# tensorchord/VectorChord-bm25

Hardware: AMD Instinct MI355X
Metric: queries/sec top-10 BM25, 10M synthetic docs; achieved HBM GB/s vs peak (higher is better)
Workload: dtype f64

## Files before the change

vectorchord-bm25_amd/api.py:

```python
import ctypes as C

import numpy as np

from ._lib import IndexDesc, SynthParams, Vbm25Error, check, lib

HIT_DTYPE = np.dtype({"names": ["score", "doc_id", "payload"],
                      "formats": ["<f8", "<u4", ("<u2", (3,))],
                      "offsets": [0, 8, 12], "itemsize": 24})

WIDTH = 16

_DESC_ARRAYS = [
    ("term_key", np.uint8), ("term_df", np.uint32), ("term_wand_fn", np.uint8),
    ("term_wand_tf", np.uint32), ("term_first_block", np.uint32), ("blk_min_doc", np.uint32),
    ("blk_max_doc", np.uint32), ("blk_n", np.uint8), ("blk_wand_fn", np.uint8),
    ("blk_wand_tf", np.uint32), ("blk_meta_doc", np.uint8), ("blk_meta_tf", np.uint8),
    ("blk_off8", np.uint32), ("blob", np.uint8), ("doc_fieldnorm", np.uint8),
    ("doc_payload", np.uint16),
]


def _p(a):
    return a.ctypes.data_as(C.c_void_p) if a is not None and a.size else None

# ... 333 lines not shown
            check(lib().vbm25_batch_set_filter(self.h, None, None))
            self.doc_filter = None
            return
        sel = np.full(self.max_queries, NO_FILTER, dtype=np.uint32)
        if q_filter is not None:
            q_filter = np.asarray(q_filter, dtype=np.uint32).reshape(-1)
            if len(q_filter) > self.max_queries:
                raise ValueError(f"{len(q_filter)} selectors for a batch of {self.max_queries} queries")
            sel[:len(q_filter)] = q_filter
        check(lib().vbm25_batch_set_filter(self.h, doc_filter.h, _p(sel)))
        self.doc_filter = doc_filter

    def set_growing(self, growing):
        check(lib().vbm25_batch_set_growing(self.h, growing.h if growing is not None else None))
        self.growing = growing

    def device_results(self):
        hits, n_hits = C.c_void_p(), C.c_void_p()
        check(lib().vbm25_batch_device_results(self.h, C.byref(hits), C.byref(n_hits)))
        return hits.value, n_hits.value

    def kernel_ms(self):
        ms, n = C.c_double(), C.c_uint32()
        check(lib().vbm25_batch_kernel_ms(self.h, C.byref(ms), C.byref(n)))
        return ms.value, n.value

    def debug_counts(self):
        f = lib().vbm25_batch_debug_counts
        f.restype = C.c_int
        f.argtypes = [C.c_void_p, C.c_void_p, C.c_void_p]
        ni, nf = C.c_uint32(), C.c_uint32()
        check(f(self.h, C.byref(ni), C.byref(nf)))
        return ni.value, nf.value

    def debug_route(self):
        f = lib().vbm25_batch_debug_route
        f.restype = C.c_int
        f.argtypes = [C.c_void_p]
        return int(f(self.h))

    def debug_routes(self):
        f = lib().vbm25_batch_debug_routes
        f.restype = C.c_int
        f.argtypes = [C.c_void_p, C.c_void_p]
        out = (C.c_uint32 * 6)()
        check(f(self.h, out))
        return tuple(int(x) for x in out)

    def debug_win_launches(self):
        f = lib().vbm25_batch_debug_win_launches
        f.restype = C.c_int
        f.argtypes = [C.c_void_p]
        return int(f(self.h))

    def debug_theta(self, nq):
        f = getattr(lib(), "vbm25_batch_debug_theta", None)
        if f is None:
            return None
        f.restype = C.c_int
        f.argtypes = [C.c_void_p, C.c_void_p]
        out = np.zeros(nq, dtype=np.uint64)
        check(f(self.h, out.ctypes.data))
        return out.view(np.float64)

    def debug_check(self):
        f = getattr(lib(), "vbm25_batch_debug_check", None)
        if f is None:
            return None
        f.restype = C.c_int
        f.argtypes = [C.c_void_p, C.c_void_p]
        out = (C.c_uint32 * 16)()
        check(f(self.h, out))
        return tuple(int(x) for x in out)


class Stream:

    def __init__(self, index, depth, max_queries, max_total_terms, k):
        self.index, self.k = index, k
        self.h = C.c_void_p()
        L = lib()
        check(L.vbm25_stream_create(index.h, depth, max_queries, max(1, max_total_terms), k, C.byref(self.h)))
        self._nq = []
        self.growing = None
        self.doc_filter = None
        self._held = []

    def __del__(self):
        try:
            if self.h:
                lib().vbm25_stream_destroy(self.h)
        except Exception:
            pass

    def set_growing(self, growing):
        check(lib().vbm25_stream_set_growing(self.h, growing.h if growing is not None else None))
        self.growing = growing

    def set_filter(self, doc_filter):
        check(lib().vbm25_stream_set_filter(self.h, doc_filter.h if doc_filter is not None else None))
        self.doc_filter = doc_filter

    def submit(self, term_ids, q_off, q_filter=None):
        term_ids = np.ascontiguousarray(term_ids, dtype=np.uint32)
        q_off = np.ascontiguousarray(q_off, dtype=np.uint32)
        nq = len(q_off) - 1
# ... 534 lines not shown
```

vectorchord-bm25_amd/csrc/scan_win.h:

```cpp

#pragma clang diagnostic push
#pragma clang diagnostic ignored "-Winline-asm"
constexpr int WN_T = 8;
#ifndef VBM25_WIN_WAVES_MAX
#define VBM25_WIN_WAVES_MAX 12
#endif
constexpr int wn_wave_lds(int mt) { return 8192 + 512 * mt + 256; }
constexpr int wn_waves(int mt, int rk) {
    const int by_lds = (163840 - 2048) / wn_wave_lds(mt);
    const int by_regs = (rk == 1 && mt <= 5) || (rk == 2 && mt <= 4) ? 16 : 12;
    const int n = by_lds < by_regs ? by_lds : by_regs;
    return n < VBM25_WIN_WAVES_MAX ? n : VBM25_WIN_WAVES_MAX;
}
constexpr int WN_BM_WORDS = 2048;
constexpr int WN_SLOT = 256;
constexpr int WN_LIST = 64;
constexpr uint32_t WN_GRID = 256;

typedef __attribute__((address_space(3))) uint32_t wn_lds_u32;
struct WnBm {
    uint32_t base, mask;
};
__device__ __forceinline__ uint32_t wn_or_rtn(const WnBm bm, const uint32_t x, const uint32_t bit) {
    return __hip_atomic_fetch_or((wn_lds_u32 *)(((x >> 3) & bm.mask) | bm.base), bit, __ATOMIC_RELAXED, __HIP_MEMORY_SCOPE_WORKGROUP);
// ... 171 lines not shown
                nsv += (uint32_t)__popcll(hm);
                continue;
            }
            if (ranked) {
                ranked = false;
                __builtin_amdgcn_wave_barrier();
                const bool hb = lane < nsv;
                rtop.offer(hb, hb ? sv_score[lane] : 0.0, hb ? sv_doc[lane] : 0u, k, lane);
            }
            rtop.offer(has, sc, d, k, lane);
        }
        __builtin_amdgcn_wave_barrier();
    }
    auto emit = [&](uint32_t i, double sc, uint32_t d) {
        const uint16_t *pl = ix.doc_payload + 3ull * d;
        unsigned long long *out = reinterpret_cast<unsigned long long *>(ca->bt.hits + (size_t)q * k + i);
        out[0] = (unsigned long long)__double_as_longlong(sc);
        out[1] = (unsigned long long)d | (unsigned long long)pl[0] << 32 | (unsigned long long)pl[1] << 48;
        out[2] = (unsigned long long)pl[2];
    };
    uint32_t n;
    if (ranked) {
        __builtin_amdgcn_wave_barrier();
        const bool mine = lane < nsv;
        const double sc = mine ? sv_score[lane] : 0.0;
        const uint32_t d = mine ? sv_doc[lane] : 0u;
        uint32_t place = 0;
        for (uint32_t j = 0; j < nsv; ++j) {
            const double sj = readlane_f64(sc, j);
            const uint32_t dj = (uint32_t)__builtin_amdgcn_readlane((int)d, (int)j);
            place += better(sj, dj, sc, d) ? 1u : 0u;
        }
        n = min(nsv, k);
        if (mine && place < k) emit(place, sc, d);
    } else {
        n = rtop.cnt;
#pragma unroll
        for (int r = 0; r < RK; ++r)
            if (r * 64 + lane < n) emit(r * 64 + lane, rtop.score[r], rtop.doc[r]);
    }
    uint32_t nf = 0;
    for (uint32_t i = lane; i < g; i += 64) {
        nf += __hip_atomic_load(&ca->bt.item_failed[L0 + i], __ATOMIC_RELAXED, __HIP_MEMORY_SCOPE_AGENT) != 0u ? 1u : 0u;
        __hip_atomic_store(&ca->bt.item_failed[L0 + i], 0u, __ATOMIC_RELAXED, __HIP_MEMORY_SCOPE_AGENT);
        __hip_atomic_store(&ca->bt.res_cnt[L0 + i], 0u, __ATOMIC_RELAXED, __HIP_MEMORY_SCOPE_AGENT);
    }
#pragma unroll
    for (int o = 32; o > 0; o >>= 1) nf += __shfl_xor(nf, o);
    if (lane == 0) {
        ca->bt.n_hits[q] = nf ? NONE32 : n;
        ca->bt.q_failed[q] = nf;
        ca->bt.theta_last[q] = theta;
        __hip_atomic_store(&ca->bt.theta[q], 0ull, __ATOMIC_RELAXED, __HIP_MEMORY_SCOPE_AGENT);
        __hip_atomic_store(&ca->bt.fused_state[1 + q], 0u, __ATOMIC_RELAXED, __HIP_MEMORY_SCOPE_AGENT);
    }
}

template <int MT, int RK, bool FILT>
__global__ void __launch_bounds__(wn_waves(MT, RK) * 64, (wn_waves(MT, RK) + 3) / 4) scan_win_kernel(DevIndex ix, DevBatch bt) {
    constexpr int WN_WAVES = wn_waves(MT, RK), WN_WG = WN_WAVES * 64;
    static_assert(sizeof(WinWave<MT>) + WN_BM_WORDS * 4 == wn_wave_lds(MT), "wn_waves() knows the size");
    __shared__ alignas(8192) uint32_t BM[WN_WAVES * WN_BM_WORDS];
    __shared__ WinWave<MT> SW[WN_WAVES];
    __shared__ double S1[256];
    const uint32_t lane = threadIdx.x & 63;
    WinWave<MT> &S = SW[uni(threadIdx.x >> 6)];
    uint32_t *const bm = &BM[uni(threadIdx.x >> 6) * WN_BM_WORDS];
    WnBm bmbase;
    bmbase.base = uni((uint32_t)(uintptr_t)(wn_lds_u32 *)bm);
    bmbase.mask = 0x1ffcu;
    asm volatile("" : "+v"(bmbase.mask));
    const uint32_t k = bt.k, g = bt.win_g, n_items = bt.nq * g, NWIN = ix.n_win;
#ifdef VBM25_DEV
    const uint32_t dbg = bt.win_dbg;
#else
    constexpr uint32_t dbg = 0;
#endif
    const uint16_t *ids16 = reinterpret_cast<const uint16_t *>(ix.post_id16);
    for (uint32_t i = threadIdx.x; i < 256u; i += WN_WG) S1[i] = ix.s1[i];
#pragma unroll
    for (int i = 0; i < WN_BM_WORDS / 4 / 64; ++i) reinterpret_cast<uint4 *>(bm)[lane + 64 * i] = make_uint4(0, 0, 0, 0);
    __syncthreads();
#ifdef VBM25_PROFILE
    unsigned long long prof[16] = {0, 0, 0, 0, 0, 0, 0, 0, 0, 0, 0, 0, 0, 0, 0, 0};
    const unsigned long long prof_t0 = __builtin_readcyclecounter();
#endif

    const uint32_t n_waves = gridDim.x * (uint32_t)WN_WAVES;
    uint32_t drawn = blockIdx.x * (uint32_t)WN_WAVES + uni(threadIdx.x >> 6);
    uint32_t merge_q = NONE32;
    if (dbg & 8u) {
        uint32_t d0 = 0;
        if (lane == 0) d0 = atomicAdd(cold_args()->bt.work_ctr, 1u);
        drawn = uni(d0);
    }
    for (;;) {
        uint32_t item = drawn;
        if (item >= n_items) break;
        uint32_t w_lo, w_hi;
        {
            const KernArgsP ca = cold_args();
            const uint32_t oo = ca->bt.order_on;
            if (oo == 1u) item = uni(ca->bt.item_order[item]);
            else if (oo == 2u) {
                const uint32_t full12 = (ca->bt.nq >> 2) * 12u;
                if (item < full12) {
                    const uint32_t wgi = item / 12u, r = item - wgi * 12u;
                    item = (wgi * 4u + (r & 3u)) * 3u + (r >> 2);
                }
            }
        }
        PROF_T(t_item);
        const uint32_t q = item / g, part = item - q * g;
        {
            const KernArgsP ca = cold_args();
            if (g <= 16u && ca->bt.win_cut[g] != 0u) {
                w_lo = ca->bt.win_cut[part];
                w_hi = ca->bt.win_cut[part + 1u];
            } else {
                w_lo = (uint32_t)((unsigned long long)NWIN * part / g);
                w_hi = (uint32_t)((unsigned long long)NWIN * (part + 1u) / g);
            }
        }

        uint32_t m = 0, term = NONE32;
        uint32_t fbi = NONE32;
        {
            const KernArgsP ca = cold_args();
            const uint32_t qs = ca->bt.q_stride;
            const uint32_t qb = qs ? qs * q : uni(ca->bt.q_off[q]), qe = qs ? qs * (q + 1u) : uni(ca->bt.q_off[q + 1]);
            const uint32_t *idfb = ca->bt.id16_fb;
            const uint32_t tt = lane < qe - qb ? ca->bt.term_ids[qb + lane] : NONE32;
            const uint32_t ti = idfb && lane < qe - qb ? idfb[qb + lane] : NONE32;
            const bool ok = tt < ix.n_terms;
            const unsigned long long okm = __ballot(ok);
            if (ok) {
                S.list[wn_mbcnt(okm)] = tt;
                if (wn_mbcnt(okm) < 32u) S.list[32u + wn_mbcnt(okm)] = ti;
            }
            m = (uint32_t)__popcll(okm);
            __builtin_amdgcn_wave_barrier();
            if (lane < min(m, (uint32_t)MT)) {
                term = S.list[lane];
                fbi = S.list[32u + lane];
            }
            __builtin_amdgcn_wave_barrier();
        }
        const bool act = lane < min(m, (uint32_t)MT);
        uint32_t fb = 0, wb = 0;
        double s0 = 0.0, kth = 0.0;
        {
            const KernArgsP ca = cold_args();
            const double *kub = ca->ix.term_kth_ub;
            if constexpr (FILT)
                if (query_filter(q)) kub = nullptr;
            if (act) {
                fb = ca->ix.term_first_block[term];
                if (fbi == NONE32) fbi = fb;
                s0 = ca->ix.term_s0[term];
                wb = ca->ix.term_win[term];
                if (kub) {
// ... 405 lines not shown
                        wn_wait_all(pb.gw);
                        c2(pb);
                    }
                    pb.found = false;
                    c1(pb, epp, nd1, w);
                    pb.valid = true;
                }
            }
#ifdef VBM25_WIN_WIPE_STORES
            if (!(dbg & 64u))
#pragma unroll
                for (int i = 0; i < WN_BM_WORDS / 4 / 64; ++i) reinterpret_cast<uint4 *>(bm)[lane + 64 * i] = make_uint4(0, 0, 0, 0);
#else
            if (!(dbg & 64u)) {
#define WN_WIPE4(o) "ds_write_addtid_b32 %1 offset:" #o "\n\tds_write_addtid_b32 %1 offset:" #o "+256\n\tds_write_addtid_b32 %1 offset:" #o "+512\n\tds_write_addtid_b32 %1 offset:" #o "+768\n\t"
#define WN_WIPE32(o) WN_WIPE4(o) WN_WIPE4(o + 1024) WN_WIPE4(o + 2048) WN_WIPE4(o + 3072) WN_WIPE4(o + 4096) WN_WIPE4(o + 5120) WN_WIPE4(o + 6144) WN_WIPE4(o + 7168)
                asm volatile("s_mov_b32 m0, %0\n\ts_nop 0\n\t" WN_WIPE32(0) : : "s"(bmbase.base), "v"(vzero) : "m0", "memory");
#undef WN_WIPE32
#undef WN_WIPE4
            }
#endif
            PROF_T(t_5);
            PROF_ADD(7, t_w2, t_5);
            {
                wn_wait_theta<MT>(pgv);
                const unsigned long long pg = ((unsigned long long)uni((uint32_t)(pgv >> 32)) << 32) | uni((uint32_t)pgv);
                if (pg > th) th = pg;
            }
            wn_load_theta(pgv, vzero, &bt.theta[q]);
            c1_request(pa);
            c1_request(pb);
            load_runs(cur, w - w_lo + 2u);
            PROF_T(t_6);
            PROF_ADD(11, t_5, t_6);
            if (failed) return false;
            return true;
        };
        PROF_T(t_loop);
        for (uint32_t w = w_lo; w < w_hi; w += 2u) {
            if (!window(bufa, w)) break;
            if (w + 1u < w_hi && !window(bufb, w + 1u)) break;
        }
        PROF_T(t_loop_end);
        double cold_ub[MT];
#pragma unroll
        for (int t = 0; t < MT; ++t) {
            const uint32_t pS = (uint32_t)__builtin_amdgcn_readlane((int)wS, t), pE = (uint32_t)__builtin_amdgcn_readlane((int)wE, t);
            const uint32_t fbt = (uint32_t)__builtin_amdgcn_readlane((int)fb, t);
            const bool in = (uint32_t)t < mm && pE != pS && (pS >> 7) + lane <= ((pE - 1u) >> 7);
            cold_ub[t] = in ? ix.blk_ub[fbt + (pS >> 7) + lane] : 0.0;
        }
        wn_drain<MT>(bufa, bufb, pa.gw, pb.gw, pgv);
        uint32_t next_draw = n_items;
        if (lane == 0 && n_items > n_waves) next_draw = atomicAdd(cold_args()->bt.work_ctr, 1u);
        if (pa.valid && !failed) c2(pa);
        if (pb.valid && !failed) c2(pb);
        failed = failed || __ballot(notf) != 0ull;

        if (!failed && !(dbg & 1u)) {
            uint32_t hm0l = 0, hm0h = 0;
#pragma unroll
            for (int t = 0; t < MT; ++t) {
                const uint32_t pS = (uint32_t)__builtin_amdgcn_readlane((int)wS, t), pE = (uint32_t)__builtin_amdgcn_readlane((int)wE, t);
                const uint32_t fbt = (uint32_t)__builtin_amdgcn_readlane((int)fb, t);
                const bool in = (uint32_t)t < mm && pE != pS && (pS >> 7) + lane <= ((pE - 1u) >> 7);
                const double ub = cold_ub[t];
                const unsigned long long hm = __ballot(in && (unsigned long long)__double_as_longlong(ub) >= th);
                if (lane == (uint32_t)t) {
                    hm0l = (uint32_t)hm;
                    hm0h = (uint32_t)(hm >> 32);
                }
            }
            for (uint32_t t = 0; t < mm; ++t) {
                const uint32_t pS = (uint32_t)__builtin_amdgcn_readlane((int)wS, (int)t), pE = (uint32_t)__builtin_amdgcn_readlane((int)wE, (int)t);
                if (pE == pS) continue;
                const uint32_t fbt = (uint32_t)__builtin_amdgcn_readlane((int)fb, (int)t);
                const double s0t = readlane_f64(s0, t);
                const uint32_t bS = pS >> 7, bE = (pE - 1u) >> 7;
                for (uint32_t b0 = bS; b0 <= bE; b0 += 64u) {
                    unsigned long long hm = (unsigned long long)(uint32_t)__builtin_amdgcn_readlane((int)hm0h, (int)t) << 32 |
                                            (uint32_t)__builtin_amdgcn_readlane((int)hm0l, (int)t);
                    if (b0 != bS) {
                        const bool in = b0 + lane <= bE;
                        double ub = 0.0;
                        if (in) ub = ix.blk_ub[fbt + b0 + lane];
                        hm = __ballot(in && (unsigned long long)__double_as_longlong(ub) >= th);
                    }
                    for (; hm != 0ull; hm &= hm - 1ull) {
                        const uint32_t blk = fbt + b0 + (uint32_t)__ffsll((long long)hm) - 1u;
                        const unsigned long long ubb = (unsigned long long)__double_as_longlong(ix.blk_ub[blk]);
                        if ((((unsigned long long)uni((uint32_t)(ubb >> 32)) << 32) | uni((uint32_t)ubb)) < th) continue;
                        const uint4 bm = uni4(ix.blk_meta[blk]);
                        const uint32_t n = bm.w & 0xff, md = (bm.w >> 8) & 0xff, mt = (bm.w >> 16) & 0xff;
                        const uint8_t *body = ix.blob + 8ull * bm.z;
                        uint32_t dd0, dd1, tt0, tt1;
                        decode_doc_ids(body, md, n, bm.x, lane, dd0, dd1);
                        decode_fields(body + ((payload_bytes(md, n) + 7u) & ~7u), mt, n, lane, tt0, tt1);
                        const uchar2 fnn = reinterpret_cast<const uchar2 *>(ix.post_fn + 128ull * blk)[lane];
#pragma nounroll
                        for (uint32_t j = 0; j < 2u; ++j) {
                            const uint32_t d = j ? dd1 : dd0, wd = d >> 16;
                            const double tf = (double)(2u * lane + j < n ? (j ? tt1 : tt0) : 1u);
                            const double sc = (tf * s0t) / (tf + S1[j ? fnn.y : fnn.x]);
                            bool cand = 2u * lane + j < n && wd >= w_lo && wd < w_hi && (unsigned long long)__double_as_longlong(sc) >= th &&
                                        (rtop.cnt < k || better(sc, d, rtop.kth_s, rtop.kth_d));
                            if (!__ballot(cand)) continue;
                            for (uint32_t t2 = 0; t2 < mm; ++t2) {
// ... 3 lines not shown
                                uint32_t lo = 0, hi = 0;
                                if (cand) {
                                    lo = ix.win_off[wb2 + wd];
                                    hi = ix.win_off[wb2 + wd + 1u];
                                }
                                while (__ballot(lo < hi)) {
                                    const uint32_t mid = (lo + hi) >> 1;
                                    if (lo < hi) {
                                        if ((uint32_t)run[mid] < (d & 0xffffu)) lo = mid + 1u;
                                        else hi = mid;
                                    }
                                }
                                if (cand && lo < ix.win_off[wb2 + wd + 1u] && (uint32_t)run[lo] == (d & 0xffffu)) cand = false;
                            }
                            offer(cand, sc, d);
                        }
                    }
                }
            }
        }
        if (rtop.cnt >= k) {
            const unsigned long long kb = (unsigned long long)__double_as_longlong(rtop.kth_s);
            if (kb > published && lane == 0) atomicMax(&bt.theta[q], kb);
        }

#ifdef VBM25_PROFILE
        {
            const unsigned long long t_end = __builtin_readcyclecounter();
            prof[12] += 1;
            prof[9] += t_loop_end - t_loop;
            prof[8] += t_loop - t_item;
            prof[13] += t_end - t_loop_end;
        }
#endif
        const uint32_t nres = failed ? 0u : rtop.cnt;
        const KernArgsP ce = cold_args();
        const size_t list = (size_t)item * ce->bt.lpi;
#pragma unroll
        for (int r = 0; r < RK; ++r)
            if (r * 64 + lane < nres) {
                __hip_atomic_store(reinterpret_cast<unsigned long long *>(&ce->bt.res_score[list * k + r * 64 + lane]),
                                   (unsigned long long)__double_as_longlong(rtop.score[r]), __ATOMIC_RELAXED, __HIP_MEMORY_SCOPE_AGENT);
                __hip_atomic_store(&ce->bt.res_doc[list * k + r * 64 + lane], rtop.doc[r], __ATOMIC_RELAXED, __HIP_MEMORY_SCOPE_AGENT);
            }
        if (lane == 0) {
            __hip_atomic_store(&ce->bt.res_cnt[list], nres, __ATOMIC_RELAXED, __HIP_MEMORY_SCOPE_AGENT);
            __hip_atomic_store(&ce->bt.item_failed[item], failed ? 0x101u : 0u, __ATOMIC_RELAXED, __HIP_MEMORY_SCOPE_AGENT);
            if (failed) *ce->bt.fail_any = 1u;
        }
        if (ce->bt.win_fuse) {
            asm volatile("s_waitcnt vmcnt(0)" ::: "memory");
            uint32_t done = 0;
            if (lane == 0) done = atomicAdd(&ce->bt.fused_state[1 + q], 1u);
            if (uni(done) == g - 1u) merge_q = q;
        }
        drawn = ((dbg & 8u) ? 0u : n_waves) + uni(next_draw);
    }
    if (merge_q != NONE32)
        wn_merge_query<RK>(ix, merge_q, g, k, lane, bm, reinterpret_cast<double *>(&S.stage[0]), reinterpret_cast<uint32_t *>(&S.stage[256]));
#ifdef VBM25_PROFILE
    if (bt.prof && lane == 0) {
        unsigned long long *o = bt.prof + ((size_t)blockIdx.x * WN_WAVES + (threadIdx.x >> 6)) * 16;
        for (int i = 0; i < 16; ++i) o[i] = prof[i];
        o[15] = __builtin_readcyclecounter() - prof_t0;
    }
#endif
}
#pragma clang diagnostic pop
```

vectorchord-bm25_amd/csrc/search.hip:

```cpp

#include <hip/hip_runtime.h>
#include <hipcub/hipcub.hpp>

#include <algorithm>
#include <atomic>
#include <cmath>
#include <cstdarg>
#include <cstdio>
#include <cstdlib>
#include <cstring>
#include <condition_variable>
#include <functional>
#include <memory>
#include <mutex>
#include <thread>
#include <string>
#include <vector>

#include "vbm25_internal.h"
#include "device_segment.h"

namespace vbm25 {

static thread_local char g_error[512] = "";
// ... 176 lines not shown
    uint64_t serial = 0;
    uint32_t n_grow = 0, n_tiles = 0, n_post = 0;
    DeviceBuffer term_start, post_g, post_c, tab_idx, tab, payload;
    std::vector<uint32_t> term_start_host;
    uint64_t device_bytes = 0;
    DeviceBuffer term_start2, post_g2, post_c2, tab_idx2, tab2;
    DeviceBuffer term_key;
    DeviceBuffer stage;
    void count_bytes() {
        device_bytes = 0;
        for (const DeviceBuffer *b : {&term_start, &post_g, &post_c, &tab_idx, &tab, &payload, &term_start2, &post_g2, &post_c2, &tab_idx2,
                                      &tab2, &term_key, &stage})
            if (b->p) device_bytes += b->bytes;
    }
    DevGrowing dev() const {
        DevGrowing g{};
        g.term_start = term_start.as<uint32_t>();
        g.post_g = post_g.as<uint32_t>();
        g.post_c = post_c.as<double>();
        g.tab_idx = tab_idx.as<uint32_t>();
        g.tab = tab.as<uint32_t>();
        g.payload = payload.as<uint16_t>();
        g.n_grow = n_grow;
        g.n_tiles = n_tiles;
        g.n_terms = index->n_terms;
        return g;
    }
};

struct Tuning {
    long long dense_x1000 = 100;
    int dense = 1;
    int ne = 1;
    int fused = 1;
    uint32_t ne_ratio = 2;
    uint32_t dense_items = D_TARGET_ITEMS;
    uint32_t range_items = R_TARGET_ITEMS, range_min_chunk = R_MIN_CHUNK_POSTINGS;
    uint32_t range_grid = R_GRID, dense_grid = D_GRID;
    uint32_t dbg = 0;
    uint32_t fused_items = 128;
    int arith = 1;
    int win = 1;
    int win_force = 0;
    uint32_t win_items = 0;
    int win_planes = 1;
    int rel16_plane = 1;
    int id16_plane = 1;
    int win_guided = 0;
    uint32_t win_grid = 0;
    int win_fuse = 1;
    int win_cut1 = 392, win_cut2 = 730;
    int win_order_arith = 1;
    int win_skew = 1;
    uint32_t id16_max_blocks = 0x00ffffff;
    uint32_t generation = 0;
};
static Tuning g_tune;
static std::mutex g_tune_mutex;
static Tuning tuning_snapshot() {
    std::lock_guard<std::mutex> g(g_tune_mutex);
    return g_tune;
}

enum class Route {
    General = 0,
    OneLaunch = 1,
    PlanFree = 2,
    Window = 3,
    Exhaustive = 4,
};

struct StagedLayout {
    size_t off = 0, dense = 0, order = 0, id16 = 0, end = 0;
    size_t sel = 0;
};
static StagedLayout staged_layout(uint32_t nq, uint32_t n_term_pos, size_t n_order, bool id16) {
    StagedLayout L;
    L.off = 4ull * n_term_pos;
    L.dense = L.off + 4ull * (nq + 1);
    L.order = L.dense + ((size_t(nq) + 7) & ~size_t(7));
    L.id16 = L.order + 4 * n_order;
    L.end = L.id16 + (id16 ? 4ull * n_term_pos : 0);
    return L;
}

static size_t pin_out_records(uint32_t nq) { return 8 + ((4ull * nq + 7) & ~size_t(7)); }

struct QueryPlan {
    Route route = Route::General;
    uint32_t g = 0;
    uint32_t win_len = 0;
    bool win_skew = false;
    bool order_identity = false;
    bool order_useful = true;
    uint32_t q_stride = 0;
    uint32_t range_mt = 0;
    bool has_dense = false;
    bool need_many = true;
    uint32_t dense_c = 0;
    uint32_t range_grid = R_GRID, dense_grid = D_GRID;
    bool id16_decode = false;
    uint64_t id16_blocks = 0;
    bool fused_pinned = false;
    uint32_t n_term_pos = 0;
    StagedLayout staged;
    uint32_t range_rt() const { return range_mt == 0 ? 0u : range_mt <= 8u ? 8u : 16u; }
};

struct vbm25_batch {
    vbm25_index *index = nullptr;
    int device = 0;
    uint32_t max_queries = 0, max_terms = 0, k = 0, nq = 0, max_items = 0;
    DeviceBuffer term_ids, q_off, items, n_items, q_item_base, theta, res_score, res_doc, res_cnt,
        hits, n_hits, error_flag, prof, q_dense, item_failed, item_order, work_ctr, hist, fused_state, dbg, fail_any, q_failed, theta_last;
    bool bigk = false;
    DeviceBuffer bk_acc, bk_keys, bk_iota, bk_docs, bk_tmp;
    size_t bk_tmp_bytes = 0;
    std::vector<uint32_t> h_terms, h_off;
    const vbm25_filter *filter = nullptr;
    DeviceBuffer filt_sel;
    std::vector<uint32_t> h_filt_sel;
    bool filt_on = false;
    const uint32_t *stage_sel = nullptr;
    const vbm25_device_growing *growing = nullptr;
    DeviceBuffer gr_sealed, gr_sealed_cnt, gr_ls, gr_lg, gr_lc, gr_acc, gr_keys, gr_iota, gr_docs, gr_tmp;
    size_t gr_tmp_bytes = 0;
    uint32_t gr_n = 0;
    std::vector<uint8_t> h_dense;
    std::vector<unsigned long long> h_postings;
    std::vector<uint32_t> h_order, h_order_q;
    Tuning tune;
    bool timing = false;
    bool use_range = false;
    uint32_t lpi = 1;
    bool use_dense = false;
    QueryPlan plan;
    DeviceBuffer id16_tmp, id16_fb;
    std::vector<uint32_t> h_id16_fb;
    DeviceBuffer qin;
    bool qin_live = false;
    bool device_consumer = false;
    bool win_nofuse = false;
    bool win_fused_run = false;
    bool state_clean = false;
    uint32_t target_items = TARGET_ITEMS;
// ... 538 lines not shown
                        const uint32_t t = term_ids[p];
                        if (t >= ixh->n_terms) continue;
                        ok = n < scan_win_max_terms() && ixh->term_win_host[t] != UINT32_MAX;
                        if (!ok) break;
                        const double e = double(ixh->term_df_host[t]) / wins;
                        ok = bt->tune.win_force || (e >= 32.0 && e <= 232.0);
                        e_max = std::max(e_max, e);
                        dfs[n++] = ixh->term_df_host[t];
                    }
                    if (ok && !bt->tune.win_force && bt->tune.ne) {
                        std::sort(dfs, dfs + n, [](uint64_t a, uint64_t b) { return a > b; });
                        uint64_t rest = 0;
                        for (uint32_t i = 0; i < n; ++i) rest += dfs[i];
                        for (uint32_t i = 0; i + 1 < n && ok; ++i) {
                            rest -= dfs[i];
                            ok = !(dfs[i] >= uint64_t(std::max(1u, bt->tune.ne_ratio)) * rest || dfs[i] * 16u >= ixh->n_docs);
                        }
                    }
                }
                if (ok) {
                    const uint32_t target = bt->tune.win_items ? bt->tune.win_items : scan_win_resident_waves(plan.range_mt, bt->k);
                    const uint32_t g_min = (ixh->n_win + 62u) / 63u;
                    const uint64_t all_win = uint64_t(nq) * ixh->n_win;
                    const uint32_t len = uint32_t(std::min<uint64_t>(63u, std::max<uint64_t>(1u, (all_win + target - 1u) / target)));
                    uint32_t gw = std::max((ixh->n_win + len - 1u) / len, g_min);
                    gw = std::min(std::min(gw, ixh->n_win), bt->max_items / nq);
                    if (gw >= g_min && gw >= 1u) {
                        win_g = gw;
                        plan.win_len = (ixh->n_win + gw - 1u) / gw > len ? 0u : len;
                    }
                }
            }
            if (win_g && !ixh->post_id16.p) {
                std::vector<uint32_t> &fbv = bt->h_id16_fb;
                fbv.resize(q_off[nq]);
                uint64_t blocks = 2;
                for (uint32_t p = 0; p < q_off[nq]; ++p) {
                    const uint32_t t = term_ids[p];
                    fbv[p] = uint32_t(std::min<uint64_t>(blocks, UINT32_MAX));
                    if (t < ixh->n_terms) blocks += (uint64_t(ixh->term_df_host[t]) + 127u) / 128u;
                }
                plan.id16_blocks = blocks;
                if (blocks > std::min<uint64_t>(bt->tune.id16_max_blocks, 0x00ffffffull)) {
                    win_g = 0;
                    plan.win_len = 0;
                }
            }
            if (bt->tune.fused && nq * g <= bt->tune.fused_items) {
                plan.route = Route::OneLaunch;
                plan.g = uint32_t(g);
                plan.fused_pinned = fast && nq <= 8 && !bt->timing;
            } else if (win_g || bt->tune.arith) {
                plan.route = win_g ? Route::Window : Route::PlanFree;
                if (win_g) g = win_g;
                plan.g = uint32_t(g);
                plan.id16_decode = win_g && !ixh->post_id16.p;
                std::vector<uint32_t> &ord = bt->h_order;
                ord.resize(size_t(nq) * g);
                std::vector<uint32_t> &qs = bt->h_order_q;
                qs.resize(nq);
                for (uint32_t q = 0; q < nq; ++q) qs[q] = q;
                {
                    unsigned long long lo = ~0ull, hi = 0;
                    for (uint32_t q = 0; q < nq; ++q) {
                        lo = std::min(lo, q_postings[q]);
                        hi = std::max(hi, q_postings[q]);
                    }
                    plan.order_identity = !(hi * 4 > lo * 5);
                    if (hi * 4 > lo * 5) std::stable_sort(qs.begin(), qs.end(), [&](uint32_t a, uint32_t b) { return q_postings[a] > q_postings[b]; });
                }

                const uint32_t wpw = win_g ? scan_win_wg(plan.range_mt, bt->k) : 0u;
                plan.win_skew = win_g == 3u && wpw == 12u && size_t(nq) * 3u <= scan_win_resident_waves(plan.range_mt, bt->k) && bt->tune.win_skew;
                plan.order_useful = plan.win_skew || (!win_g || !bt->tune.win_guided ? q_postings[qs[0]] * 4 > q_postings[qs[nq - 1]] * 5 : true) ||
                                 (win_g && size_t(nq) * win_g > scan_win_resident_waves(plan.range_mt, bt->k));
                if (plan.win_skew) {
                    const uint32_t full = nq / 4u;
                    for (uint32_t wgi = 0; wgi < full; ++wgi)
                        for (uint32_t s4 = 0; s4 < 4u; ++s4)
                            for (uint32_t part = 0; part < 3u; ++part) ord[size_t(wgi) * 12u + part * 4u + s4] = qs[wgi * 4u + s4] * 3u + part;
                    for (uint32_t qi = full * 4u; qi < nq; ++qi)
                        for (uint32_t part = 0; part < 3u; ++part) ord[size_t(qi) * 3u + part] = qs[qi] * 3u + part;
                } else if (win_g)
                    for (uint32_t part = 0; part < g; ++part)
                        for (uint32_t i = 0; i < nq; ++i) ord[size_t(part) * nq + i] = qs[i] * uint32_t(g) + part;
                else
                for (uint32_t i = 0; i < nq; ++i)
                    for (uint32_t part = 0; part < g; ++part) ord[size_t(i) * g + part] = qs[i] * uint32_t(g) + part;
            }
        }
    }
    const bool with_order = plan.route == Route::PlanFree || plan.route == Route::Window;
    plan.staged = staged_layout(nq, q_off[nq], with_order ? size_t(nq) * plan.g : 0, plan.id16_decode);
    if (nq && q_off[1] != 0) {
        plan.q_stride = q_off[1];
        for (uint32_t q = 0; q < nq && plan.q_stride; ++q)
            if (q_off[q + 1] - q_off[q] != plan.q_stride) plan.q_stride = 0;
    }
    const uint32_t dense_target = std::max(256u, bt->tune.dense_items);
    plan.dense_c = plan.has_dense ? std::max(1u, (dense_target + n_dense / 2) / std::max(n_dense, 1u)) : 0u;
    if (plan.has_dense) {
        const uint32_t floor_c = std::max(std::max(1u, 4096u / std::max(n_dense, 1u)), ixh->n_docs >> 16);
        if (bt->tune.dense_items == D_TARGET_ITEMS) plan.dense_c = std::min(plan.dense_c, floor_c);
    }
    unsigned long long sparse_postings = 0;
    for (uint32_t q = 0; q < nq; ++q)
        if (!(plan.dense_c && dense[q])) sparse_postings += q_postings[q];
    unsigned long long chunk = (sparse_postings + bt->target_items - 1) / bt->target_items;
    if (chunk < bt->min_chunk) chunk = bt->min_chunk;
    unsigned long long items = 0;
    for (uint32_t q = 0; q < nq; ++q) {
        if (!q_postings[q]) continue;
        if (plan.dense_c && dense[q]) {
            items += std::min(plan.dense_c, ixh->n_docs);
            continue;
        }
        unsigned long long c = (q_postings[q] + chunk / 2) / chunk;
        if (c == 0) c = 1;
        if (c > ixh->n_docs) c = ixh->n_docs;
        items += c;
    }
    plan.range_grid = uint32_t(std::min<unsigned long long>(std::max<unsigned long long>(items, 1), std::max(1u, bt->tune.range_grid)));
    plan.dense_grid = uint32_t(std::min<unsigned long long>(std::max<unsigned long long>(items, 1), std::max(1u, bt->tune.dense_grid)));
#ifdef VBM25_PROFILE
    plan.range_grid = std::min<uint32_t>(plan.range_grid, R_GRID);
#endif
}

static int commit_queries(vbm25_batch *bt, const uint32_t *term_ids, const uint32_t *q_off, uint32_t nq, bool fast, const QueryPlan &plan) {
    if (int rc = use_device(bt->index->device)) return rc;
    if (plan.route == Route::Exhaustive) {
        bt->h_terms.assign(term_ids, term_ids + q_off[nq]);
        bt->h_off.assign(q_off, q_off + nq + 1);
    } else {
        if (plan.id16_decode) {
// ... 221 lines not shown
    HIP_TRY(hipGetLastError());
    return VBM25_OK;
}

static int run_one_launch(vbm25_batch *bt, hipStream_t st, DevBatch db) {
    const QueryPlan &plan = bt->plan;
    const DevIndex &ix = bt->index->dev;
    if (int rc = reset_launch_state(bt, st, true)) return rc;
    db.fused_g = plan.g;
    db.dense_on = 0;
    if (plan.fused_pinned) {
        db.term_ids = reinterpret_cast<const uint32_t *>(bt->pin_in);
        db.q_off = reinterpret_cast<const uint32_t *>(bt->pin_in + plan.staged.off);
        if (bt->filt_on && plan.staged.sel) db.filt_sel = reinterpret_cast<const uint32_t *>(bt->pin_in + plan.staged.sel);
        db.n_hits = reinterpret_cast<uint32_t *>(bt->pin_out + 8);
        db.hits = reinterpret_cast<vbm25_hit *>(bt->pin_out + pin_out_records(bt->nq));
    }
    hipEvent_t e1;
    if (int rc = take_events(bt, st, e1)) return rc;
    const uint32_t fgrid = std::min<uint32_t>(bt->nq * plan.g, R_GRID);
    const int rcf = dispatch_k(bt->k, [&](auto kmax) {
        constexpr int KM = decltype(kmax)::value;
        if constexpr (KM <= REG_K) {
            if (plan.range_rt() == 8) scan_range_kernel<KM, 8, true><<<fgrid, RWG, 0, st>>>(ix, db);
            else scan_range_kernel<KM, 16, true><<<fgrid, RWG, 0, st>>>(ix, db);
            if (!plan.fused_pinned) {
                scan_many_kernel<KM><<<std::min<uint32_t>(bt->nq * plan.g, TARGET_ITEMS), WG, 0, st>>>(ix, db);
                if (bt->timing) (void)hipEventRecord(e1, st);
                DevBatch dm = db;
                dm.merge_marked = 1;
                merge_kernel<KM><<<bt->nq, 64, 0, st>>>(ix, dm);
            } else if (bt->timing) {
                (void)hipEventRecord(e1, st);
            }
        }
        return int(VBM25_OK);
    });
    if (rcf) return rcf;
    HIP_TRY(hipGetLastError());
    bt->state_clean = true;
    return VBM25_OK;
}

static int run_window(vbm25_batch *bt, hipStream_t st, DevBatch db) {
    const QueryPlan &plan = bt->plan;
    const DevIndex &ix = bt->index->dev;
    if (int rc = reset_launch_state(bt, st, false)) return rc;
    db.fused_g = plan.g;
    db.win_g = plan.g;
    {
        const uint32_t gq = plan.g, nwin = bt->index->n_win;
        std::memset(db.win_cut, 0, sizeof db.win_cut);
        if (plan.win_skew) {
            db.win_cut[0] = 0;
            db.win_cut[1] = uint32_t(uint64_t(nwin) * uint32_t(bt->tune.win_cut1) / 1000u);
            db.win_cut[2] = uint32_t(uint64_t(nwin) * uint32_t(bt->tune.win_cut2) / 1000u);
            db.win_cut[3] = nwin;
            if (db.win_cut[1] > 63u || db.win_cut[2] - db.win_cut[1] > 63u || nwin - db.win_cut[2] > 63u) std::memset(db.win_cut, 0, sizeof db.win_cut);
        } else if (gq <= 16u && plan.win_len && uint64_t(plan.win_len) * (gq - 1u) < nwin) {
            for (uint32_t p = 0; p < gq; ++p) db.win_cut[p] = plan.win_len * p;
            db.win_cut[gq] = nwin;
        }
    }
    db.lpi = 1;
    db.hist = nullptr;
    db.dense_on = 0;
    db.many_expected = 0;
    db.merge_clean = 1;
    db.order_on = plan.order_useful ? (plan.win_skew && plan.order_identity && bt->tune.win_order_arith ? 2u : 1u) : 0u;
    db.q_stride = plan.q_stride;
    hipEvent_t e1;
    if (int rc = take_events(bt, st, e1)) return rc;
    const uint32_t wmt = std::min(plan.range_mt, 8u), wpw = scan_win_wg(wmt, bt->k);
    const uint32_t wgrid = std::min<uint32_t>((bt->nq * plan.g + wpw - 1u) / wpw, bt->tune.win_grid ? bt->tune.win_grid : scan_win_resident_waves(wmt, bt->k) / wpw);
    const bool fuse = bt->tune.win_fuse && !bt->win_nofuse && !bt->device_consumer && !bt->growing && uint64_t(bt->nq) * plan.g <= scan_win_resident_waves(wmt, bt->k) && !bt->tune.win_grid;
    db.win_fuse = fuse ? 1u : 0u;
    bt->win_fused_run = fuse;
    if (plan.id16_decode) {
        const StagedLayout &L = plan.staged;
        db.id16_fb = bt->id16_fb.as<uint32_t>();
        if (bt->qin_live && (L.sel ? L.sel : L.end) > L.id16) db.id16_fb = reinterpret_cast<const uint32_t *>(bt->qin.as<uint8_t>() + L.id16);
        if (plan.n_term_pos) decode_id16_kernel<<<plan.n_term_pos, DI_WAVES * 64, 0, st>>>(ix, db.term_ids, db.id16_fb, bt->id16_tmp.as<uint32_t>());
        DevIndex ixw = ix;
        ixw.post_id16 = bt->id16_tmp.as<uint32_t>();
        HIP_TRY(scan_win_launch(ixw, db, wmt, wgrid, st));
    } else
    HIP_TRY(scan_win_launch(ix, db, wmt, wgrid, st));
    if (fuse) {
        if (bt->timing) (void)hipEventRecord(e1, st);
    } else
    (void)dispatch_k(bt->k, [&](auto kmax) {
        constexpr int KM = decltype(kmax)::value;
        if constexpr (KM <= REG_K) {
            scan_many_kernel<KM><<<64, WG, 0, st>>>(ix, db);
            if (bt->timing) (void)hipEventRecord(e1, st);
            merge_kernel<KM><<<bt->nq, 64, 0, st>>>(ix, db);
        }
        return int(VBM25_OK);
    });
    HIP_TRY(hipGetLastError());
    bt->state_clean = true;
    return VBM25_OK;
}

static int run_plan_free(vbm25_batch *bt, hipStream_t st, DevBatch db) {
    const QueryPlan &plan = bt->plan;
    const DevIndex &ix = bt->index->dev;
    if (int rc = reset_launch_state(bt, st, false)) return rc;
    db.fused_g = plan.g;
    db.dense_on = 0;
    db.many_expected = 0;
    db.merge_clean = 1;
    db.order_on = 1;
    hipEvent_t e1;
    if (int rc = take_events(bt, st, e1)) return rc;
    const uint32_t agrid = std::min<uint32_t>(bt->nq * plan.g, std::max(1u, bt->tune.range_grid));
    const int rca = dispatch_k(bt->k, [&](auto kmax) {
        constexpr int KM = decltype(kmax)::value;
        if constexpr (KM <= REG_K) {
            if (plan.range_rt() == 8) scan_range_kernel<KM, 8><<<agrid, RWG, 0, st>>>(ix, db);
            else scan_range_kernel<KM, 16><<<agrid, RWG, 0, st>>>(ix, db);
            scan_many_kernel<KM><<<64, WG, 0, st>>>(ix, db);
            if (bt->timing) (void)hipEventRecord(e1, st);
            merge_kernel<KM><<<bt->nq, 64, 0, st>>>(ix, db);
        }
        return int(VBM25_OK);
    });
    if (rca) return rca;
// ... 190 lines not shown
    a.n_terms = ix->n_terms;
    a.q_terms = dq.as<uint32_t>();
    a.doc_start = ds.as<uint64_t>();
    a.doc_term = dt.as<uint32_t>();
    a.doc_tf = df.as<uint32_t>();
    a.term_idf = ix->term_idf.as<double>();
    a.s1 = ix->dev.s1;
    a.fn_len = ix->fn_len.as<uint32_t>();
    a.k1p1 = ix->k1 + 1.0;
    a.out = dout.as<double>();
    evaluate_kernel<<<(n_docs + 255) / 256, 256>>>(a);
    HIP_TRY(hipGetLastError());
    HIP_TRY(hipMemcpy(scores, dout.p, 8ull * n_docs, hipMemcpyDeviceToHost));
    return VBM25_OK;
}

int vbm25_evaluate_batch(vbm25_index *ix, const uint32_t *q_terms, uint32_t n_q, uint32_t n_docs,
                         const uint64_t *doc_start, const uint32_t *doc_term, const uint32_t *doc_tf, double *scores) {
    return guarded([&] { return vbm25_evaluate_batch_impl(ix, q_terms, n_q, n_docs, doc_start, doc_term, doc_tf, scores); });
}

int vbm25_tuning_set(const char *name, long long value) {
    if (!name) return set_error(VBM25_ERR_INVALID, "NULL argument");
    std::lock_guard<std::mutex> guard(g_tune_mutex);
    const std::string n(name);
    if (n == "dense_x1000") g_tune.dense_x1000 = value;
    else if (n == "dense") g_tune.dense = value != 0;
    else if (n == "ne") g_tune.ne = value != 0;
    else if (n == "fused") g_tune.fused = value != 0;
    else if (n == "ne_ratio") g_tune.ne_ratio = (uint32_t)std::max(1ll, value);
    else if (n == "dense_items") g_tune.dense_items = (uint32_t)std::max(256ll, value);
    else if (n == "range_items") g_tune.range_items = (uint32_t)std::max(256ll, value);
    else if (n == "range_min_chunk") g_tune.range_min_chunk = (uint32_t)std::max(128ll, value);
    else if (n == "range_grid") g_tune.range_grid = (uint32_t)std::max(1ll, value);
    else if (n == "dense_grid") g_tune.dense_grid = (uint32_t)std::max(1ll, value);
#ifdef VBM25_DEV
    else if (n == "dbg") g_tune.dbg = (uint32_t)value;
#endif
    else if (n == "fused_items") g_tune.fused_items = (uint32_t)std::max(0ll, value);
    else if (n == "arith") g_tune.arith = value != 0;
    else if (n == "win") g_tune.win = value != 0;
    else if (n == "win_force") g_tune.win_force = value != 0;
    else if (n == "win_items") g_tune.win_items = (uint32_t)std::max(0ll, value);
    else if (n == "win_planes") g_tune.win_planes = value != 0;
    else if (n == "win_guided") g_tune.win_guided = value != 0;
    else if (n == "rel16_plane") g_tune.rel16_plane = value != 0;
    else if (n == "id16_plane") g_tune.id16_plane = value != 0;
    else if (n == "win_order_arith") g_tune.win_order_arith = value != 0;
    else if (n == "win_grid") g_tune.win_grid = (uint32_t)std::max(0ll, value);
    else if (n == "win_skew") g_tune.win_skew = value != 0;
    else if (n == "win_cut1") g_tune.win_cut1 = int(std::min<long long>(std::max<long long>(value, 1), 998));
    else if (n == "win_cut2") g_tune.win_cut2 = int(std::min<long long>(std::max<long long>(value, 2), 999));
    else if (n == "win_fuse") g_tune.win_fuse = value != 0;
    else if (n == "id16_max_blocks") g_tune.id16_max_blocks = (uint32_t)std::min<long long>(std::max(2ll, value), 0x00ffffffll);
    else return set_error(VBM25_ERR_INVALID, "unknown tuning switch %s", name);
    ++g_tune.generation;
    return VBM25_OK;
}
void vbm25_tuning_reset(void) {
    std::lock_guard<std::mutex> guard(g_tune_mutex);
    const uint32_t gen = g_tune.generation + 1u;
    g_tune = Tuning();
    g_tune.generation = gen;
}

static bool plan_free_kernels(const vbm25_batch *bt) { return bt->plan.route == Route::PlanFree || bt->plan.route == Route::Window; }

int vbm25_batch_debug_counts(vbm25_batch *bt, uint32_t *n_items, uint32_t *n_failed) {
    if (!bt || !n_items || !n_failed) return set_error(VBM25_ERR_INVALID, "NULL argument");
    *n_items = *n_failed = 0;
    if (bt->bigk) return VBM25_OK;
    if (int rc = use_device(bt->index->device)) return rc;
    HIP_TRY(hipStreamSynchronize(bt->last_stream));
    if (plan_free_kernels(bt) && bt->state_clean) {
        *n_items = bt->nq * bt->plan.g;
        std::vector<uint32_t> qf(bt->nq);
        if (bt->nq) HIP_TRY(hipMemcpy(qf.data(), bt->q_failed.p, 4ull * bt->nq, hipMemcpyDeviceToHost));
        *n_failed = 0;
        for (uint32_t x : qf) *n_failed += x;
        return VBM25_OK;
    }
    HIP_TRY(hipMemcpy(n_items, bt->n_items.p, 4, hipMemcpyDeviceToHost));
    std::vector<uint32_t> f(*n_items);
    if (*n_items) HIP_TRY(hipMemcpy(f.data(), bt->item_failed.p, 4ull * *n_items, hipMemcpyDeviceToHost));
    *n_failed = 0;
    for (uint32_t x : f) *n_failed += x != 0;
    return VBM25_OK;
}

int vbm25_batch_debug_route(vbm25_batch *bt) {
    if (!bt) return -1;
    return int(bt->bigk ? Route::Exhaustive : bt->plan.route);
}

int vbm25_batch_debug_routes(vbm25_batch *bt, uint32_t *out6) {
    if (!bt || !out6) return set_error(VBM25_ERR_INVALID, "NULL argument");
    for (int i = 0; i < 6; ++i) out6[i] = 0;
    if (bt->bigk) return VBM25_OK;
    if (int rc = use_device(bt->index->device)) return rc;
    HIP_TRY(hipStreamSynchronize(bt->last_stream));
    for (uint32_t q = 0; q < bt->nq; ++q) out6[bt->h_dense[q] ? 1 : 0]++;
    if (bt->plan.route == Route::General) {
        uint32_t n = 0;
        HIP_TRY(hipMemcpy(&n, bt->n_items.p, 4, hipMemcpyDeviceToHost));
        n = std::min(n, bt->max_items);
        std::vector<Item> items(n);
        if (n) HIP_TRY(hipMemcpy(items.data(), bt->items.p, sizeof(Item) * size_t(n), hipMemcpyDeviceToHost));
        for (const Item &it : items) {
            const uint32_t m = it.m & ~ITEM_DENSE;
            out6[3 + (m > 16u ? 2 : (it.m & ITEM_DENSE) ? 1 : 0)]++;
        }
    }
    return VBM25_OK;
}

int vbm25_batch_debug_win_launches(vbm25_batch *bt) {
    if (!bt || bt->plan.route != Route::Window) return 0;
    return bt->win_fused_run ? 1 : 3;
}

int vbm25_batch_debug_check(vbm25_batch *bt, uint32_t *out4) {
    if (!bt || !out4) return set_error(VBM25_ERR_INVALID, "NULL argument");
    if (int rc = use_device(bt->index->device)) return rc;
    HIP_TRY(hipStreamSynchronize(bt->last_stream));
    if (!bt->dbg.p) {
        std::memset(out4, 0, 64);
        return VBM25_OK;
    }
    HIP_TRY(hipMemcpy(out4, bt->dbg.p, 64, hipMemcpyDeviceToHost));
    HIP_TRY(hipMemset(bt->dbg.p, 0, 64));
    return VBM25_OK;
}

int vbm25_batch_debug_theta(vbm25_batch *bt, unsigned long long *out) {
    if (!bt || !out) return set_error(VBM25_ERR_INVALID, "NULL argument");
    if (int rc = use_device(bt->index->device)) return rc;
    HIP_TRY(hipStreamSynchronize(bt->last_stream));
    if (bt->nq && bt->theta.p)
        HIP_TRY(hipMemcpy(out, plan_free_kernels(bt) && bt->state_clean ? bt->theta_last.p : bt->theta.p, 8ull * bt->nq, hipMemcpyDeviceToHost));
    return VBM25_OK;
}

int vbm25_batch_set_timing(vbm25_batch *bt, int enabled) {
    if (!bt) return set_error(VBM25_ERR_INVALID, "batch is NULL");
    bt->timing = enabled != 0;
    bt->events_used = 0;
    return VBM25_OK;
}

int vbm25_batch_kernel_ms(vbm25_batch *bt, double *avg_ms, uint32_t *n_launches) {
    if (!bt || !avg_ms) return set_error(VBM25_ERR_INVALID, "NULL argument");
    if (int rc = use_device(bt->index->device)) return rc;
    double sum = 0;
    for (size_t i = 0; i < bt->events_used; ++i) {
        HIP_TRY(hipEventSynchronize(bt->events[i].second));
        float ms = 0;
        HIP_TRY(hipEventElapsedTime(&ms, bt->events[i].first, bt->events[i].second));
        sum += ms;
    }
    *avg_ms = bt->events_used ? sum / double(bt->events_used) : 0.0;
    if (n_launches) *n_launches = uint32_t(bt->events_used);
    bt->events_used = 0;
    return VBM25_OK;
}

#ifdef VBM25_PROFILE
int vbm25_batch_profile(vbm25_batch *bt, unsigned long long *out, uint32_t n_workgroups) {
    HIP_TRY(hipDeviceSynchronize());
    HIP_TRY(hipMemcpy(out, bt->prof.p, 8ull * 16 * RNW * std::min<uint32_t>(n_workgroups, R_GRID), hipMemcpyDeviceToHost));
    return VBM25_OK;
}
// ... 1362 lines not shown
```

Measured before the change: 5.871 million.

## Allow fused window kernel beyond resident waves and add optional rest-window pool

Removes the restriction that the fused window launch requires all items to fit in resident waves. To make that work, the last worker resets the work counter and queries ready to merge are chained through fused_state as a linked list that the wave drains. It also adds an optional split of the tail windows into extra pooled parts (off by default) with matching item-order remapping, plus a debug accessor for items. The risk is correctness in the merge chaining and grid sizing when the fused path now runs non-resident.

```diff
diff --git a/vectorchord-bm25_amd/api.py b/vectorchord-bm25_amd/api.py
--- a/vectorchord-bm25_amd/api.py
+++ b/vectorchord-bm25_amd/api.py
@@ -409,6 +409,16 @@
         f.restype = C.c_int
         f.argtypes = [C.c_void_p]
         return int(f(self.h))
+
+    def debug_items(self):
+        f = lib().vbm25_batch_debug_items
+        f.restype = C.c_int
+        f.argtypes = [C.c_void_p, C.c_void_p, C.c_uint32, C.c_void_p]
+        n = self.debug_counts()[0]
+        items = np.zeros((n, 4), dtype=np.uint32)
+        base = np.zeros(self.nq + 1, dtype=np.uint32)
+        check(f(self.h, items.ctypes.data, n, base.ctypes.data))
+        return items, base
 
     def debug_theta(self, nq):
         f = getattr(lib(), "vbm25_batch_debug_theta", None)
diff --git a/vectorchord-bm25_amd/csrc/scan_win.h b/vectorchord-bm25_amd/csrc/scan_win.h
--- a/vectorchord-bm25_amd/csrc/scan_win.h
+++ b/vectorchord-bm25_amd/csrc/scan_win.h
@@ -247,7 +247,6 @@
         ca->bt.q_failed[q] = nf;
         ca->bt.theta_last[q] = theta;
         __hip_atomic_store(&ca->bt.theta[q], 0ull, __ATOMIC_RELAXED, __HIP_MEMORY_SCOPE_AGENT);
-        __hip_atomic_store(&ca->bt.fused_state[1 + q], 0u, __ATOMIC_RELAXED, __HIP_MEMORY_SCOPE_AGENT);
     }
 }
 
@@ -298,10 +297,22 @@
             const uint32_t oo = ca->bt.order_on;
             if (oo == 1u) item = uni(ca->bt.item_order[item]);
             else if (oo == 2u) {
-                const uint32_t full12 = (ca->bt.nq >> 2) * 12u;
+                const uint32_t nqs = ca->bt.nq, full12 = (nqs >> 2) * 12u;
                 if (item < full12) {
                     const uint32_t wgi = item / 12u, r = item - wgi * 12u;
-                    item = (wgi * 4u + (r & 3u)) * 3u + (r >> 2);
+                    item = (wgi * 4u + (r & 3u)) * g + (r >> 2);
+                } else if (g != 3u) {
+                    if (item < nqs * 3u) {
+                        const uint32_t qq = item / 3u;
+                        item = qq * g + (item - qq * 3u);
+                    } else {
+                        uint32_t r = item - nqs * 3u, pp = 3u;
+                        while (r >= nqs) {
+                            r -= nqs;
+                            ++pp;
+                        }
+                        item = r * g + pp;
+                    }
                 }
             }
         }
@@ -813,7 +824,12 @@
         }
         wn_drain<MT>(bufa, bufb, pa.gw, pb.gw, pgv);
         uint32_t next_draw = n_items;
-        if (lane == 0 && n_items > n_waves) next_draw = atomicAdd(cold_args()->bt.work_ctr, 1u);
+        if (lane == 0 && n_items > n_waves) {
+            const KernArgsP ca = cold_args();
+            next_draw = atomicAdd(ca->bt.work_ctr, 1u);
+            if (ca->bt.win_fuse && next_draw + 1u == n_items + ((dbg & 8u) ? n_waves : 0u))
+                __hip_atomic_store(ca->bt.work_ctr, 0u, __ATOMIC_RELAXED, __HIP_MEMORY_SCOPE_AGENT);
+        }
         if (pa.valid && !failed) c2(pa);
         if (pb.valid && !failed) c2(pb);
         failed = failed || __ballot(notf) != 0ull;
@@ -923,12 +939,21 @@
             asm volatile("s_waitcnt vmcnt(0)" ::: "memory");
             uint32_t done = 0;
             if (lane == 0) done = atomicAdd(&ce->bt.fused_state[1 + q], 1u);
-            if (uni(done) == g - 1u) merge_q = q;
+            if (uni(done) == g - 1u) {
+                if (lane == 0) __hip_atomic_store(&ce->bt.fused_state[1 + q], merge_q, __ATOMIC_RELAXED, __HIP_MEMORY_SCOPE_AGENT);
+                merge_q = q;
+            }
         }
         drawn = ((dbg & 8u) ? 0u : n_waves) + uni(next_draw);
     }
-    if (merge_q != NONE32)
+    while (merge_q != NONE32) {
+        uint32_t *const link = &cold_args()->bt.fused_state[1 + merge_q];
+        uint32_t next_q = 0;
+        if (lane == 0) next_q = __hip_atomic_load(link, __ATOMIC_RELAXED, __HIP_MEMORY_SCOPE_AGENT);
         wn_merge_query<RK>(ix, merge_q, g, k, lane, bm, reinterpret_cast<double *>(&S.stage[0]), reinterpret_cast<uint32_t *>(&S.stage[256]));
+        merge_q = uni(next_q);
+        if (lane == 0) __hip_atomic_store(link, 0u, __ATOMIC_RELAXED, __HIP_MEMORY_SCOPE_AGENT);
+    }
 #ifdef VBM25_PROFILE
     if (bt.prof && lane == 0) {
         unsigned long long *o = bt.prof + ((size_t)blockIdx.x * WN_WAVES + (threadIdx.x >> 6)) * 16;
diff --git a/vectorchord-bm25_amd/csrc/search.hip b/vectorchord-bm25_amd/csrc/search.hip
--- a/vectorchord-bm25_amd/csrc/search.hip
+++ b/vectorchord-bm25_amd/csrc/search.hip
@@ -252,6 +252,8 @@
     int win_cut1 = 392, win_cut2 = 730;
     int win_order_arith = 1;
     int win_skew = 1;
+    int win_rest = 0;
+    int win_rest_parts = 1;
     uint32_t id16_max_blocks = 0x00ffffff;
     uint32_t generation = 0;
 };
@@ -291,6 +293,8 @@
     uint32_t g = 0;
     uint32_t win_len = 0;
     bool win_skew = false;
+    uint32_t win_rest = 0;
+    uint32_t win_pool = 0;
     bool order_identity = false;
     bool order_useful = true;
     uint32_t q_stride = 0;
@@ -935,6 +939,17 @@
                 plan.fused_pinned = fast && nq <= 8 && !bt->timing;
             } else if (win_g || bt->tune.arith) {
                 plan.route = win_g ? Route::Window : Route::PlanFree;
+                const uint32_t wpw = win_g ? scan_win_wg(plan.range_mt, bt->k) : 0u;
+                plan.win_skew = win_g == 3u && wpw == 12u && size_t(nq) * 3u <= scan_win_resident_waves(plan.range_mt, bt->k) && bt->tune.win_skew;
+                if (plan.win_skew && bt->tune.win_rest > 0) {
+                    const uint32_t parts = uint32_t(bt->tune.win_rest_parts);
+                    const uint32_t rest = std::max(parts, uint32_t(uint64_t(ixh->n_win) * uint32_t(bt->tune.win_rest) / 1000u));
+                    if (rest + 3u <= ixh->n_win && uint64_t(nq) * (3u + parts) <= bt->max_items) {
+                        plan.win_rest = rest;
+                        plan.win_pool = parts;
+                        win_g = 3u + parts;
+                    }
+                }
                 if (win_g) g = win_g;
                 plan.g = uint32_t(g);
                 plan.id16_decode = win_g && !ixh->post_id16.p;
@@ -953,17 +968,17 @@
                     if (hi * 4 > lo * 5) std::stable_sort(qs.begin(), qs.end(), [&](uint32_t a, uint32_t b) { return q_postings[a] > q_postings[b]; });
                 }
 
-                const uint32_t wpw = win_g ? scan_win_wg(plan.range_mt, bt->k) : 0u;
-                plan.win_skew = win_g == 3u && wpw == 12u && size_t(nq) * 3u <= scan_win_resident_waves(plan.range_mt, bt->k) && bt->tune.win_skew;
                 plan.order_useful = plan.win_skew || (!win_g || !bt->tune.win_guided ? q_postings[qs[0]] * 4 > q_postings[qs[nq - 1]] * 5 : true) ||
                                  (win_g && size_t(nq) * win_g > scan_win_resident_waves(plan.range_mt, bt->k));
                 if (plan.win_skew) {
-                    const uint32_t full = nq / 4u;
+                    const uint32_t full = nq / 4u, gi = uint32_t(g);
                     for (uint32_t wgi = 0; wgi < full; ++wgi)
                         for (uint32_t s4 = 0; s4 < 4u; ++s4)
-                            for (uint32_t part = 0; part < 3u; ++part) ord[size_t(wgi) * 12u + part * 4u + s4] = qs[wgi * 4u + s4] * 3u + part;
+                            for (uint32_t part = 0; part < 3u; ++part) ord[size_t(wgi) * 12u + part * 4u + s4] = qs[wgi * 4u + s4] * gi + part;
                     for (uint32_t qi = full * 4u; qi < nq; ++qi)
-                        for (uint32_t part = 0; part < 3u; ++part) ord[size_t(qi) * 3u + part] = qs[qi] * 3u + part;
+                        for (uint32_t part = 0; part < 3u; ++part) ord[size_t(qi) * 3u + part] = qs[qi] * gi + part;
+                    for (uint32_t part = 3u; part < gi; ++part)
+                        for (uint32_t qi = 0; qi < nq; ++qi) ord[size_t(part) * nq + qi] = qs[qi] * gi + part;
                 } else if (win_g)
                     for (uint32_t part = 0; part < g; ++part)
                         for (uint32_t i = 0; i < nq; ++i) ord[size_t(part) * nq + i] = qs[i] * uint32_t(g) + part;
@@ -1291,11 +1306,15 @@
         const uint32_t gq = plan.g, nwin = bt->index->n_win;
         std::memset(db.win_cut, 0, sizeof db.win_cut);
         if (plan.win_skew) {
+            const uint32_t body = nwin - plan.win_rest;
             db.win_cut[0] = 0;
-            db.win_cut[1] = uint32_t(uint64_t(nwin) * uint32_t(bt->tune.win_cut1) / 1000u);
-            db.win_cut[2] = uint32_t(uint64_t(nwin) * uint32_t(bt->tune.win_cut2) / 1000u);
-            db.win_cut[3] = nwin;
-            if (db.win_cut[1] > 63u || db.win_cut[2] - db.win_cut[1] > 63u || nwin - db.win_cut[2] > 63u) std::memset(db.win_cut, 0, sizeof db.win_cut);
+            db.win_cut[1] = uint32_t(uint64_t(body) * uint32_t(bt->tune.win_cut1) / 1000u);
+            db.win_cut[2] = uint32_t(uint64_t(body) * uint32_t(bt->tune.win_cut2) / 1000u);
+            db.win_cut[3] = body;
+            for (uint32_t p = 1; p <= plan.win_pool; ++p) db.win_cut[3u + p] = body + uint32_t(uint64_t(plan.win_rest) * p / plan.win_pool);
+            bool fits = true;
+            for (uint32_t p = 0; p < gq; ++p) fits = fits && db.win_cut[p + 1u] - db.win_cut[p] <= 63u;
+            if (!fits) std::memset(db.win_cut, 0, sizeof db.win_cut);
         } else if (gq <= 16u && plan.win_len && uint64_t(plan.win_len) * (gq - 1u) < nwin) {
             for (uint32_t p = 0; p < gq; ++p) db.win_cut[p] = plan.win_len * p;
             db.win_cut[gq] = nwin;
@@ -1311,8 +1330,8 @@
     hipEvent_t e1;
     if (int rc = take_events(bt, st, e1)) return rc;
     const uint32_t wmt = std::min(plan.range_mt, 8u), wpw = scan_win_wg(wmt, bt->k);
-    const uint32_t wgrid = std::min<uint32_t>((bt->nq * plan.g + wpw - 1u) / wpw, bt->tune.win_grid ? bt->tune.win_grid : scan_win_resident_waves(wmt, bt->k) / wpw);
-    const bool fuse = bt->tune.win_fuse && !bt->win_nofuse && !bt->device_consumer && !bt->growing && uint64_t(bt->nq) * plan.g <= scan_win_resident_waves(wmt, bt->k) && !bt->tune.win_grid;
+    const uint32_t wgrid = std::min<uint32_t>((bt->nq * (plan.g - plan.win_pool) + wpw - 1u) / wpw, bt->tune.win_grid ? bt->tune.win_grid : scan_win_resident_waves(wmt, bt->k) / wpw);
+    const bool fuse = bt->tune.win_fuse && !bt->win_nofuse && !bt->device_consumer && !bt->growing;
     db.win_fuse = fuse ? 1u : 0u;
     bt->win_fused_run = fuse;
     if (plan.id16_decode) {
@@ -1609,6 +1628,8 @@
     else if (n == "win_cut1") g_tune.win_cut1 = int(std::min<long long>(std::max<long long>(value, 1), 998));
     else if (n == "win_cut2") g_tune.win_cut2 = int(std::min<long long>(std::max<long long>(value, 2), 999));
     else if (n == "win_fuse") g_tune.win_fuse = value != 0;
+    else if (n == "win_rest") g_tune.win_rest = int(std::min<long long>(std::max<long long>(value, 0), 500));
+    else if (n == "win_rest_parts") g_tune.win_rest_parts = int(std::min<long long>(std::max<long long>(value, 1), 2));
     else if (n == "id16_max_blocks") g_tune.id16_max_blocks = (uint32_t)std::min<long long>(std::max(2ll, value), 0x00ffffffll);
     else return set_error(VBM25_ERR_INVALID, "unknown tuning switch %s", name);
     ++g_tune.generation;
@@ -1674,6 +1695,18 @@
 int vbm25_batch_debug_win_launches(vbm25_batch *bt) {
     if (!bt || bt->plan.route != Route::Window) return 0;
     return bt->win_fused_run ? 1 : 3;
+}
+
+int vbm25_batch_debug_items(vbm25_batch *bt, uint32_t *items, uint32_t cap, uint32_t *q_item_base) {
+    if (!bt || !items || !q_item_base) return set_error(VBM25_ERR_INVALID, "NULL argument");
+    if (!plan_free_kernels(bt)) return set_error(VBM25_ERR_INVALID, "the current queries' route keeps no item records of this kind");
+    const uint64_t n = uint64_t(bt->nq) * bt->plan.g;
+    if (n > cap) return set_error(VBM25_ERR_INVALID, "%llu items exceed the caller's %u", (unsigned long long)n, cap);
+    if (int rc = use_device(bt->index->device)) return rc;
+    HIP_TRY(hipStreamSynchronize(bt->last_stream));
+    if (n) HIP_TRY(hipMemcpy(items, bt->items.p, sizeof(Item) * n, hipMemcpyDeviceToHost));
+    HIP_TRY(hipMemcpy(q_item_base, bt->q_item_base.p, 4ull * (bt->nq + 1), hipMemcpyDeviceToHost));
+    return VBM25_OK;
 }
 
 int vbm25_batch_debug_check(vbm25_batch *bt, uint32_t *out4) {
```

Result: no change. 5.888 million, median of 6 (+0.3%).
